# bcc-research/CFMMRouter.jl

Measured on AMD Instinct MI355X. Metric: find_arb! pools/sec + route! wall-clock, 1M-pool arbitrage, 1/2/4/8 GPU, higher is better.
Workload: dtype f64; 1 GPU; config3: 1M mixed ProductTwoCoin + GeometricMeanTwoCoin pools (500k each), 256 tokens, LinearNonnegative arbitrage; pools_per_gpu=1000000, pools_total=1000000, variant=materialising, full=False

## Files before the change

### cfmmrouter.jl_amd/csrc/sweep_core.h

```cpp
#pragma once

#include "granule.h"
#include "ops_two_coin.h"
#include "ops_univ3.h"

#include <type_traits>

namespace cfmm {

typedef double d2v __attribute__((ext_vector_type(2)));
__device__ __forceinline__ void store_pair(double2* dst, double x, double y, int nt)
{
    d2v val = {x, y};
    if (nt) asm volatile("global_store_dwordx4 %0, %1, off nt\n\ts_nop 1" : : "v"(dst), "v"(val) : "memory");
    else asm volatile("global_store_dwordx4 %0, %1, off sc1\n\ts_nop 1" : : "v"(dst), "v"(val) : "memory");
}
__device__ __forceinline__ void store_pair_at(double2* base, uint32_t i, double x, double y)
{
    d2v val = {x, y};
    asm volatile("s_nop 4\n\tglobal_store_dwordx4 %0, %1, %2 sc1\n\ts_nop 1" : : "v"(i * 16u), "v"(val), "s"(base) : "memory");
}

__device__ __forceinline__ void store_row(double* dst, double x)
{
    asm volatile("global_store_dwordx2 %0, %1, off sc1" : : "v"(dst), "v"(x) : "memory");
}

struct SweepLds {
    double2* vy;
    double2* gtab;
    double* lv;
    double* bins;
    double* wsum;
    double* flags;
    double* my_bins;
};

template <int BLOCK, bool GBINS>
__device__ __forceinline__ SweepLds carve_lds(const SweepArgs& a)
{
    extern __shared__ __attribute__((aligned(16))) double lds[];
    SweepLds L;
    if constexpr (GBINS) {
        L.vy = nullptr;
        L.gtab = nullptr;
        L.lv = L.bins = L.my_bins = L.flags = nullptr;
        L.wsum = lds;
        return L;
    }
    L.vy = reinterpret_cast<double2*>(lds);
    L.gtab = reinterpret_cast<double2*>(lds + ((size_t)a.n_pad << (a.v_shift - 3)));
    L.lv = reinterpret_cast<double*>(L.gtab + a.gtab_n);
    L.bins = L.lv + (a.need_logv ? a.n_pad : 0);
    L.wsum = L.bins + (size_t)a.copies * a.n_pad;
    L.flags = L.wsum + BLOCK / 64;
    L.my_bins = L.bins + (size_t)(a.copies == 1 ? 0 : (threadIdx.x >> 6)) * a.n_pad;
    return L;
}

__device__ __forceinline__ int wait_armed(const SweepArgs& a)
{
    const long long t0 = (long long)wall_clock64();
    for (;;) {
        const unsigned long long w = __hip_atomic_load(a.arm_word, __ATOMIC_RELAXED, __HIP_MEMORY_SCOPE_SYSTEM);
        if (w == a.arm_seq) return 1;
        if ((w & ~kArmCancel) > a.arm_seq || w == (a.arm_seq | kArmCancel)) return 0;
        if ((long long)wall_clock64() - t0 > a.arm_timeout) return -1;
        __builtin_amdgcn_s_sleep(1);
    }
}

__device__ __forceinline__ void report(const SweepArgs& a, unsigned long long bit)
{
    if (a.flags && threadIdx.x == 0) __hip_atomic_fetch_or(a.flags, bit, __ATOMIC_RELAXED, __HIP_MEMORY_SCOPE_SYSTEM);
}

constexpr int kStageLive = 1, kStageFast = 2, kStageGaveUp = 4;
constexpr int kPricePre = 2;
struct PricePre {
    double p[kPricePre];
};
template <int BLOCK>
__device__ __forceinline__ PricePre request_prices(const double* v, int n)
{
    PricePre r;
#pragma unroll
    for (int k = 0; k < kPricePre; ++k) {
        const int j = (int)threadIdx.x + k * BLOCK;
        r.p[k] = v[j < n ? j : n - 1];
    }
    return r;
}
template <int BLOCK, bool GBINS, bool PRE = false, bool LEAN = false>
__device__ __forceinline__ int stage_prices(const SweepArgs& a, const SweepLds& L, const PricePre& pre = PricePre{})
{
    if constexpr (GBINS) {
        __syncthreads();
        return kStageLive;
    }
    const int tid = threadIdx.x;
    const int n_zero = a.copies * a.n_pad;
    const bool logs = a.need_logv != 0;
    const bool armed = a.arm_word != nullptr;
    bool live = true, gave_up = false;
    if (armed) {
        for (int j = tid; j < n_zero; j += BLOCK) L.bins[j] = 0.0;
        for (int j = tid; j < a.gtab_n; j += BLOCK) {
            const double g = a.gtab[j];
            L.gtab[j] = make_double2(g, rcp_refined(g));
        }
        if (tid == 0) L.flags[BLOCK / 64] = (double)wait_armed(a);
        __syncthreads();
        live = L.flags[BLOCK / 64] > 0.0;
        gave_up = L.flags[BLOCK / 64] < 0.0;
    }
    bool in_window = true;
    for (int j = tid, k = 0; j < a.n; j += BLOCK, ++k) {
        double vj;
        if (armed) vj = __hip_atomic_load(a.v + j, __ATOMIC_RELAXED, __HIP_MEMORY_SCOPE_SYSTEM);
        else if (PRE && k < kPricePre) vj = k == 0 ? pre.p[0] : pre.p[1];
        else vj = a.v[j];
        if (a.v_shift == 4) L.vy[j] = make_double2(vj, rcp_refined(vj));
        else reinterpret_cast<double*>(L.vy)[j] = vj;
        in_window = in_window && in_fast_window(vj);
        if (logs) L.lv[j] = log(vj);
    }
    if (!armed) {
        for (int j = tid; j < n_zero; j += BLOCK) L.bins[j] = 0.0;
        for (int j = tid; j < a.gtab_n; j += BLOCK) {
            const double g = a.gtab[j];
            L.gtab[j] = make_double2(g, rcp_refined(g));
        }
    }
    const bool wave_in = __all(in_window ? 1 : 0) != 0;
    if ((tid & 63) == 0) L.flags[tid >> 6] = wave_in ? 1.0 : 0.0;
    __syncthreads();
    bool all_in = true;
    if constexpr (LEAN) {
        static_assert((BLOCK / 64) % 2 == 0, "flags are read in pairs");
        const double2* pairs = reinterpret_cast<const double2*>(L.flags);
        int bits = -1;
#pragma unroll
        for (int w = 0; w < BLOCK / 128; ++w) {
            const double2 f = pairs[w];
            bits &= __double2hiint(f.x) & __double2hiint(f.y);
        }
        all_in = bits != 0;
    } else {
#pragma unroll
        for (int w = 0; w < BLOCK / 64; ++w) all_in = all_in && L.flags[w] != 0.0;
    }
    return (live ? kStageLive : 0) | (all_in ? kStageFast : 0) | (gave_up ? kStageGaveUp : 0);
}

template <class Ops, bool MAT, bool GBINS, bool FAST, bool LEAN, class Idx>
__device__ __forceinline__ void finish_pool(const Ops& ops, const SweepArgs& a, const SweepLds& L, const typename Ops::Raw& raw,
                                            const Px& px, int2 tok, Idx i, double& acc)
{
    const auto put_record = [&](double x, double y) {
        if constexpr (LEAN) store_pair_at(a.Delta, i, x, y);
        else store_pair(a.Delta + i, x, y, a.nt_stores);
    };
    Trade t;
    double d, l;
    int dir;
    dir = ops.template solve_dir<FAST>(raw, px, d, l, t);
    const double v1 = px.v1, v2 = px.v2;
    const bool one = dir == kDir1 || dir == kDir2;
    const bool plain = one && (!MAT || !a.compact || (__double2hiint(d) | __double2hiint(l)) >= 0);
    if (plain) {
        const bool d1 = dir == kDir1;
        if (MAT) {
            if (a.compact) {
                put_record(d1 ? d : -d, l);
            } else {
                store_pair(a.Delta + i, d1 ? d : 0.0, d1 ? 0.0 : d, a.nt_stores);
                store_pair(a.Lambda + i, d1 ? 0.0 : l, d1 ? l : 0.0, a.nt_stores);
            }
        }
        acc += l * (d1 ? v2 : v1) - d * (d1 ? v1 : v2);
        if constexpr (GBINS) {
            a.gflow[i] = d1 ? make_double2(0.0 - d, l) : make_double2(l, 0.0 - d);
        } else {
            const double f_in = 0.0 - d;
            if (f_in != 0.0) atomicAdd(&L.my_bins[d1 ? tok.x : tok.y], f_in);
            if (l != 0.0) atomicAdd(&L.my_bins[d1 ? tok.y : tok.x], l);
        }
        return;
    }
    if (dir == kDirNone) {
        if (MAT) {
            if (a.compact) {
                put_record(0.0, 0.0);
            } else {
                store_pair(a.Delta + i, 0.0, 0.0, a.nt_stores);
                store_pair(a.Lambda + i, 0.0, 0.0, a.nt_stores);
            }
        }
        if constexpr (GBINS) a.gflow[i] = make_double2(0.0, 0.0);
        return;
    }
    expand_dir(dir, d, l, t);
    if (MAT) {
        if (a.compact) {
            const int d1h = __double2hiint(t.d1), d2h = __double2hiint(t.d2), l1h = __double2hiint(t.l1), l2h = __double2hiint(t.l2);
            const int z1 = d2h | __double2loint(t.d2) | l1h | __double2loint(t.l1);
            const int z2 = d1h | __double2loint(t.d1) | l2h | __double2loint(t.l2);
            const bool dir1 = (z1 == 0) & ((d1h | l2h) >= 0);
            const bool dir2 = (z2 == 0) & ((d2h | l1h) >= 0);
            double ra = t.d1, rb = t.l2;
            if (!dir1) {
                if (dir2) {
                    ra = -t.d2;
                    rb = t.l1;
                } else {
                    a.Lambda[i] = make_double2(t.d1, t.d2);
                    a.Over[i] = make_double2(t.l1, t.l2);
                    ra = 0.0;
                    rb = -1.0;
                }
            }
            put_record(ra, rb);
        } else {
            store_pair(a.Delta + i, t.d1, t.d2, a.nt_stores);
            store_pair(a.Lambda + i, t.l1, t.l2, a.nt_stores);
        }
    }
    acc += (t.l1 * v1 + t.l2 * v2) - (t.d1 * v1 + t.d2 * v2);
    const double f1 = t.l1 - t.d1, f2 = t.l2 - t.d2;
    if constexpr (GBINS) {
        a.gflow[i] = make_double2(f1, f2);
    } else {
        if (f1 != 0.0) atomicAdd(&L.my_bins[tok.x], f1);
        if (f2 != 0.0) atomicAdd(&L.my_bins[tok.y], f2);
    }
}

template <class Ops> struct HasLeanSolve : std::false_type {};
template <> struct HasLeanSolve<ProductOps> : std::true_type {};
template <> struct HasLeanSolve<GeoMeanLogOps> : std::true_type {};

template <class Ops, bool MAT, bool FAST, class Idx>
__device__ __forceinline__ void process_pool_lean(const Ops& ops, const SweepArgs& a, const SweepLds& L,
                                                  const typename Ops::Raw& raw_in, Idx i, double& acc)
{
    typename Ops::Raw raw = raw_in;
    const unsigned packed = (unsigned)raw.ai.x;
    const int2 tok = make_int2((int)(packed & 0xffffu), (int)(packed >> 16));
    const double2 gy = L.gtab[ops.p.gbase + raw.ai.y];
    const double2 a1 = L.vy[tok.x], a2 = L.vy[tok.y];
    double g = gy.x, yg = gy.y, v1 = a1.x, y1 = a1.y, v2 = a2.x, y2 = a2.y, lv1 = 0.0, lv2 = 0.0;
    if constexpr (Ops::kNeedsLogPrices) {
        lv1 = L.lv[tok.x];
        lv2 = L.lv[tok.y];
        asm volatile("" : "+v"(g), "+v"(yg), "+v"(v1), "+v"(y1), "+v"(v2), "+v"(y2), "+v"(lv1), "+v"(lv2));
    } else {
        asm volatile("" : "+v"(g), "+v"(yg), "+v"(v1), "+v"(y1), "+v"(v2), "+v"(y2));
    }
    raw.ai = tok;
    raw.g = g;
    raw.yg = yg;
    const Px px{v1, v2, y1, y2, yg, lv2 - lv1};
    double d, l;
    bool dir1, trades, rare;
    ops.template lean_solve<FAST>(raw, px, d, l, dir1, trades, rare);
    if (MAT) rare = rare | ((__double2hiint(d) | __double2hiint(l)) < 0);
    if (__builtin_expect(__any(rare ? 1 : 0) != 0, 0)) {
        finish_pool<Ops, MAT, false, FAST, true>(ops, a, L, raw, px, tok, i, acc);
        return;
    }
    if (MAT) store_pair_at(a.Delta, i, dir1 ? d : -d, l);
    const double worth = l * (dir1 ? v2 : v1) - d * (dir1 ? v1 : v2);
    acc = trades ? acc + worth : acc;
    const double f_in = 0.0 - d;
    if (f_in != 0.0) atomicAdd(&L.my_bins[dir1 ? tok.x : tok.y], f_in);
    if (l != 0.0) atomicAdd(&L.my_bins[dir1 ? tok.y : tok.x], l);
}

template <class Ops, bool MAT, bool GBINS, bool FAST, bool LEAN, class Idx>
__device__ __forceinline__ void process_pool(const Ops& ops, const SweepArgs& a, const SweepLds& L,
                                             const typename Ops::Raw& raw_in, Idx i, double& acc)
{
    if constexpr (LEAN && HasLeanSolve<Ops>::value) {
        process_pool_lean<Ops, MAT, FAST>(ops, a, L, raw_in, i, acc);
        return;
    }
    typename Ops::Raw raw = raw_in;
    ops.template resolve<GBINS, FAST, LEAN>(raw, L.gtab);
    const int2 tok = ops.tokens(raw);
    Px px;
    px.yg = raw.yg;
    if constexpr (GBINS) {
        px.v1 = a.v[tok.x];
        px.v2 = a.v[tok.y];
        px.y1 = px.y2 = 0.0;
        px.dlv = Ops::kNeedsLogPrices ? log(px.v2 / px.v1) : 0.0;
    } else {
        if constexpr (FAST) {
            const double2 a1 = L.vy[tok.x], a2 = L.vy[tok.y];
            px.v1 = a1.x; px.y1 = a1.y;
            px.v2 = a2.x; px.y2 = a2.y;
        } else {
            const char* base = reinterpret_cast<const char*>(L.vy);
            px.v1 = *reinterpret_cast<const double*>(base + ((size_t)tok.x << a.v_shift));
            px.v2 = *reinterpret_cast<const double*>(base + ((size_t)tok.y << a.v_shift));
            px.y1 = px.y2 = 0.0;
        }
        px.dlv = 0.0;
        if constexpr (Ops::kNeedsLogPrices)
            px.dlv = a.need_logv ? L.lv[tok.y] - L.lv[tok.x] : log(px.v2 / px.v1);
    }
    finish_pool<Ops, MAT, GBINS, FAST, LEAN>(ops, a, L, raw, px, tok, i, acc);
}

template <class Ops, bool MAT, int BLOCK, bool GBINS, bool FAST, bool PREFETCH, bool LEAN, class Idx>
__device__ __forceinline__ void tile_loop(const Ops& ops, const SweepArgs& a, const SweepLds& L, typename Ops::Raw cur,
                                          Idx i, Idx step, Idx left, double& acc)
{
    if constexpr (PREFETCH) {
        bool ok = left > 0;
        while (ok) {
            const bool more = left > 1;
            typename Ops::Raw nxt = cur;
            if (more) nxt = ops.template load<GBINS, LEAN>((Idx)(i + step));
            process_pool<Ops, MAT, GBINS, FAST, LEAN>(ops, a, L, cur, i, acc);
            i += step;
            --left;
            ok = more;
            cur = nxt;
        }
    } else {
        bool ok = left > 0;
        while (ok) {
            process_pool<Ops, MAT, GBINS, FAST, LEAN>(ops, a, L, cur, i, acc);
            i += step;
            ok = --left > 0;
            if (ok) cur = ops.template load<GBINS, LEAN>(i);
        }
    }
}

constexpr int kArithFull = 0, kArithFast = 1, kArithAuto = 2;
template <class Ops, bool MAT, int BLOCK, bool GBINS, int FASTK, bool MULTI, bool LEAN, class Idx>
__device__ __forceinline__ double sweep_tiles(const Ops& ops, const SweepArgs& a, const SweepLds& L, const typename Ops::Raw& cur,
                                              Idx i, Idx step, Idx left, bool& poison, bool& live, const PricePre& pre)
{
    static_assert(!(GBINS && FASTK != kArithFull), "large-market mode runs on the compiler's sequences");
    double acc = 0.0;
    const int staged = stage_prices<BLOCK, GBINS, !GBINS, LEAN>(a, L, pre);
    poison = (staged & kStageLive) == 0;
    live = !poison || (staged & kStageGaveUp) != 0;
    if (staged & kStageGaveUp) report(a, kFlagGaveUp);
    if (FASTK == kArithFast && !poison && (staged & kStageFast) == 0) {
        poison = true;
        report(a, kFlagWindow);
    }
    if (poison) left = 0;
    constexpr bool kPre = Ops::kPrefetch && !MULTI;
    if constexpr (FASTK == kArithAuto) {
        if (staged & kStageFast) tile_loop<Ops, MAT, BLOCK, GBINS, true, kPre, LEAN>(ops, a, L, cur, i, step, left, acc);
        else tile_loop<Ops, MAT, BLOCK, GBINS, false, kPre, LEAN>(ops, a, L, cur, i, step, left, acc);
    } else {
        tile_loop<Ops, MAT, BLOCK, GBINS, FASTK == kArithFast, kPre, LEAN>(ops, a, L, cur, i, step, left, acc);
    }
    return acc;
}

typedef unsigned long long u2v __attribute__((ext_vector_type(2)));
__device__ __forceinline__ void publish_column(const SweepArgs& a, int j, double val)
{
    if (a.direct_host.gran) {
        u2v g = {granule(a.direct_host.tag, val, 0), granule(a.direct_host.tag, val, 1)};
        asm volatile("global_store_dwordx4 %0, %1, off sc0 sc1\n\ts_nop 1" : : "v"(a.direct_host.gran + 2 * (size_t)j), "v"(g) : "memory");
    } else {
        a.direct_out[j] = val;
    }
}

template <int BLOCK, bool GBINS>
__device__ __forceinline__ void finish_row(const SweepArgs& a, const SweepLds& L, double acc, int row_id, bool poison, bool publish)
{
    const double nan = __builtin_nan("");
    if (poison) acc = nan;
    constexpr int kWaves = BLOCK / 64;
    const int tid = threadIdx.x;
    const int wave = tid >> 6;
#pragma unroll
    for (int off = 32; off > 0; off >>= 1) acc += __shfl_down(acc, off, 64);
    if ((tid & 63) == 0) L.wsum[wave] = acc;
    __syncthreads();

    const int n_cols = GBINS ? 0 : a.n;
    if (!GBINS && a.direct) {
        if (!publish) return;
        for (int j = tid; j < n_cols; j += BLOCK) {
            double s = L.bins[j];
            for (int c = 1; c < a.copies; ++c) s += L.bins[(size_t)c * a.n_pad + j];
            publish_column(a, j, poison ? nan : s);
        }
        if (tid == 0) {
            double s = L.wsum[0];
            for (int w = 1; w < kWaves; ++w) s += L.wsum[w];
            publish_column(a, n_cols, poison ? nan : s);
        }
        return;
    }
    double* row = a.partials + (size_t)row_id * a.row_pitch;
    for (int j = tid; j < n_cols; j += BLOCK) {
        double s = L.bins[j];
        for (int c = 1; c < a.copies; ++c) s += L.bins[(size_t)c * a.n_pad + j];
        store_row(row + j, poison ? nan : s);
    }
    if (tid == 0) {
        double s = L.wsum[0];
        for (int w = 1; w < kWaves; ++w) s += L.wsum[w];
        store_row(row + n_cols, poison ? nan : s);
    }
}

#define CFMM_CONST_AS __attribute__((address_space(4)))
template <class T>
__device__ __forceinline__ const CFMM_CONST_AS T* const_as(const T* p)
{
    return (const CFMM_CONST_AS T*)(reinterpret_cast<uintptr_t>(p));
}
struct LaunchHead {
    const SweepDesc* desc;
    const double* v;
    int reverse;
    int n;
};
static_assert(offsetof(SweepLaunch, desc) == 0 && offsetof(SweepLaunch, v) == 8 && offsetof(SweepLaunch, reverse) == 16 &&
                  offsetof(SweepLaunch, n) == 20 && offsetof(SweepLaunch, tail) == 24 && alignof(SweepTail) == 8,
              "sweep_kernel / sweep_multi (pointer, pointer, int, int, SweepTail) read the segment as a SweepLaunch");
typedef const CFMM_CONST_AS SweepLaunch& LaunchRef;
__device__ __forceinline__ LaunchRef launch_args()
{
    return *(const CFMM_CONST_AS SweepLaunch*)__builtin_amdgcn_kernarg_segment_ptr();
}
__device__ __forceinline__ BlockRec block_rec(const SweepDesc* desc)
{
    const CFMM_CONST_AS BlockRec* recs =
        (const CFMM_CONST_AS BlockRec*)(reinterpret_cast<uintptr_t>(desc) + kSweepDescHead);
    const CFMM_CONST_AS BlockRec& r = recs[blockIdx.x];
    return BlockRec{r.first, r.stride, r.full, r.tail, r.row, r.seg, r.kind};
}
__device__ __forceinline__ SweepArgs block_args(const LaunchHead& h, LaunchRef la, const CFMM_CONST_AS SweepDesc& d,
                                                const CFMM_CONST_AS SegRec& sg)
{
    const CFMM_CONST_AS SweepTail& t = la.tail;
    SweepArgs a;
    a.v = la.v;
    a.n = d.n;
    a.n_pad = d.n_pad;
    a.v_shift = d.v_shift;
    a.need_logv = d.need_logv;
    a.gtab = d.gtab;
    a.gtab_n = d.gtab_n;
    a.copies = d.copies;
    a.flags = d.flags;
    a.m = sg.m;
    a.Delta = sg.Delta;
    a.Lambda = sg.Lambda;
    a.Over = sg.Over;
    a.compact = d.compact;
    a.partials = d.partials;
    a.row_pitch = d.row_pitch;
    a.gflow = sg.gflow;
    a.reverse = h.reverse;
    a.arm_word = t.arm_word;
    a.arm_seq = t.arm_seq;
    a.arm_timeout = t.arm_timeout;
    a.nt_stores = d.nt_stores;
    a.direct = d.direct;
    a.direct_out = t.direct_out;
    a.direct_host = HostOut{t.direct_host.gran, t.direct_host.tag};
    return a;
}
__device__ __forceinline__ ProductPools pools_of(const CFMM_CONST_AS AnyPools& u, const ProductPools*)
{
    return ProductPools{u.p.R, u.p.gamma, u.p.Ai, u.p.pk, u.p.gbase};
}
__device__ __forceinline__ GeoMeanPools pools_of(const CFMM_CONST_AS AnyPools& u, const GeoMeanPools*)
{
    return GeoMeanPools{u.g.R, u.g.w, u.g.gamma, u.g.Ai, u.g.eta, u.g.Q, u.g.reference_order, u.g.pk, u.g.gbase};
}
__device__ __forceinline__ UniV3Pools pools_of(const CFMM_CONST_AS AnyPools& u, const UniV3Pools*)
{
    return UniV3Pools{u.u.pg, u.u.Ai, u.u.cur_a, u.u.cur_b, u.u.cur_c, u.u.curR, u.u.walk, u.u.ticks, u.u.thr, u.u.head,
                      u.u.has_walk, u.u.cp, u.u.pk, u.u.gbase};
}
template <class Ops, bool MAT, int BLOCK, bool GBINS, int FASTK, bool MULTI, bool LEAN>
__device__ __forceinline__ void sweep_body(const LaunchHead& h, const CFMM_CONST_AS SweepDesc& d, const CFMM_CONST_AS SegRec& sg,
                                           const BlockRec& br, const PricePre& pre)
{
    static_assert(!(LEAN && (GBINS || FASTK == kArithFull)), "the lean kernels: LDS bins, prices staged as pairs");
    using Idx = typename std::conditional<LEAN, uint32_t, int64_t>::type;
    const Ops ops{pools_of(sg.pools, (const decltype(Ops::p)*)nullptr)};
    const int64_t stride = br.stride;
    const int64_t i0 = br.first + threadIdx.x;
    const int64_t left = br.full + ((int)threadIdx.x < br.tail ? 1 : 0);
    const bool reverse = h.reverse != 0;
    const int64_t step = reverse ? -stride : stride;
    const int64_t i = reverse ? i0 + (left - 1) * stride : i0;
    typename Ops::Raw cur = {};
    if (left > 0) cur = ops.template load<GBINS, LEAN>((Idx)i);
    SweepArgs a = block_args(h, launch_args(), d, sg);
    if constexpr (LEAN) {
        a.compact = 1;
        a.nt_stores = 0;
        a.v_shift = 4;
        a.copies = BLOCK / 64;
        a.direct = 0;
    }
    const SweepLds L = carve_lds<BLOCK, GBINS>(a);
    if constexpr (LEAN) a.need_logv = Ops::kNeedsLogPrices ? 1 : 0;
    bool poison, live;
    const double acc = sweep_tiles<Ops, MAT, BLOCK, GBINS, FASTK, MULTI, LEAN>(ops, a, L, cur, (Idx)i, (Idx)step, (Idx)left, poison, live, pre);
    finish_row<BLOCK, GBINS>(a, L, acc, br.row, poison, live);
}

template <class Ops, bool MAT, int BLOCK, bool GBINS, int FASTK, bool LEAN = false>
__global__ __launch_bounds__(BLOCK) void sweep_kernel(const SweepDesc* desc, const double* v, int reverse, int n, SweepTail)
{
    const LaunchHead h{desc, v, reverse, n};
    PricePre pre = {};
    if constexpr (!GBINS) pre = request_prices<BLOCK>(v, n);
    const BlockRec br = block_rec(desc);
    const CFMM_CONST_AS SweepDesc& d = *const_as(desc);
    sweep_body<Ops, MAT, BLOCK, GBINS, FASTK, false, LEAN>(h, d, d.seg[0], br, pre);
}

template <bool MAT, int BLOCK, bool GBINS, int FASTK, bool LEAN = false>
__global__ __launch_bounds__(BLOCK) void sweep_multi(const SweepDesc* desc, const double* v, int reverse, int n, SweepTail)
{
    const LaunchHead h{desc, v, reverse, n};
    PricePre pre = {};
    if constexpr (!GBINS) pre = request_prices<BLOCK>(v, n);
    const BlockRec br = block_rec(desc);
    const CFMM_CONST_AS SweepDesc& d = *const_as(desc);
    const CFMM_CONST_AS SegRec& sg = d.seg[br.seg];
    switch (br.kind) {
    case 0: sweep_body<ProductOps, MAT, BLOCK, GBINS, FASTK, true, LEAN>(h, d, sg, br, pre); break;
    case 1:
        sweep_body<GeoMeanLogOps, MAT, BLOCK, GBINS, FASTK, true, LEAN>(h, d, sg, br, pre);
        break;
    default: sweep_body<UniV3Ops, MAT, BLOCK, GBINS, FASTK, true, LEAN>(h, d, sg, br, pre); break;
    }
}
#undef CFMM_CONST_AS

}
```

Measured before the change: 83.04 billion pools/s.

## Prefetch fee table at kernel entry and hand-schedule vmem waits in sweep loop

```diff
diff --git a/cfmmrouter.jl_amd/csrc/sweep_core.h b/cfmmrouter.jl_amd/csrc/sweep_core.h
--- a/cfmmrouter.jl_amd/csrc/sweep_core.h
+++ b/cfmmrouter.jl_amd/csrc/sweep_core.h
@@ -91,8 +91,22 @@
     }
     return r;
 }
+struct FeePre {
+    double g;
+};
+template <int BLOCK, bool LEAN>
+__device__ __forceinline__ FeePre request_fee(const double* gtab, int gtab_n)
+{
+    static_assert(kMaxFeeTable <= BLOCK, "the fee table is one entry per lane");
+    FeePre r = {1.0};
+    const int last = gtab_n - 1, j = (int)threadIdx.x;
+    if (LEAN || last >= 0) r.g = gtab[j < last ? j : last];
+    return r;
+}
+__device__ __forceinline__ void wait_vmem() { __builtin_amdgcn_s_waitcnt(0x0f70); }
 template <int BLOCK, bool GBINS, bool PRE = false, bool LEAN = false>
-__device__ __forceinline__ int stage_prices(const SweepArgs& a, const SweepLds& L, const PricePre& pre = PricePre{})
+__device__ __forceinline__ int stage_prices(const SweepArgs& a, const SweepLds& L, const PricePre& pre = PricePre{},
+                                            const FeePre& fee = FeePre{})
 {
     if constexpr (GBINS) {
         __syncthreads();
@@ -103,12 +117,19 @@
     const bool logs = a.need_logv != 0;
     const bool armed = a.arm_word != nullptr;
     bool live = true, gave_up = false;
+    const auto stage_fee = [&] {
+        if constexpr (PRE) {
+            if (tid < a.gtab_n) L.gtab[tid] = make_double2(fee.g, rcp_refined(fee.g));
+        } else {
+            for (int j = tid; j < a.gtab_n; j += BLOCK) {
+                const double g = a.gtab[j];
+                L.gtab[j] = make_double2(g, rcp_refined(g));
+            }
+        }
+    };
     if (armed) {
         for (int j = tid; j < n_zero; j += BLOCK) L.bins[j] = 0.0;
-        for (int j = tid; j < a.gtab_n; j += BLOCK) {
-            const double g = a.gtab[j];
-            L.gtab[j] = make_double2(g, rcp_refined(g));
-        }
+        stage_fee();
         if (tid == 0) L.flags[BLOCK / 64] = (double)wait_armed(a);
         __syncthreads();
         live = L.flags[BLOCK / 64] > 0.0;
@@ -117,8 +138,10 @@
     bool in_window = true;
     for (int j = tid, k = 0; j < a.n; j += BLOCK, ++k) {
         double vj;
-        if (armed) vj = __hip_atomic_load(a.v + j, __ATOMIC_RELAXED, __HIP_MEMORY_SCOPE_SYSTEM);
-        else if (PRE && k < kPricePre) vj = k == 0 ? pre.p[0] : pre.p[1];
+        if (armed) {
+            vj = __hip_atomic_load(a.v + j, __ATOMIC_RELAXED, __HIP_MEMORY_SCOPE_SYSTEM);
+            if constexpr (PRE) wait_vmem();
+        } else if (PRE && k < kPricePre) vj = k == 0 ? pre.p[0] : pre.p[1];
         else vj = a.v[j];
         if (a.v_shift == 4) L.vy[j] = make_double2(vj, rcp_refined(vj));
         else reinterpret_cast<double*>(L.vy)[j] = vj;
@@ -127,10 +150,7 @@
     }
     if (!armed) {
         for (int j = tid; j < n_zero; j += BLOCK) L.bins[j] = 0.0;
-        for (int j = tid; j < a.gtab_n; j += BLOCK) {
-            const double g = a.gtab[j];
-            L.gtab[j] = make_double2(g, rcp_refined(g));
-        }
+        stage_fee();
     }
     const bool wave_in = __all(in_window ? 1 : 0) != 0;
     if ((tid & 63) == 0) L.flags[tid >> 6] = wave_in ? 1.0 : 0.0;
@@ -317,25 +337,33 @@
 __device__ __forceinline__ void tile_loop(const Ops& ops, const SweepArgs& a, const SweepLds& L, typename Ops::Raw cur,
                                           Idx i, Idx step, Idx left, double& acc)
 {
+    wait_vmem();
     if constexpr (PREFETCH) {
         bool ok = left > 0;
-        while (ok) {
-            const bool more = left > 1;
+        for (;;) {
+            const bool more = ok && left > 1;
+            if (__any(more ? 1 : 0) == 0) break;
             typename Ops::Raw nxt = cur;
             if (more) nxt = ops.template load<GBINS, LEAN>((Idx)(i + step));
-            process_pool<Ops, MAT, GBINS, FAST, LEAN>(ops, a, L, cur, i, acc);
+            if (ok) process_pool<Ops, MAT, GBINS, FAST, LEAN>(ops, a, L, cur, i, acc);
             i += step;
             --left;
             ok = more;
             cur = nxt;
         }
+        if (MAT) __builtin_amdgcn_s_waitcnt(0x0f71);
+        else wait_vmem();
+        if (ok) process_pool<Ops, MAT, GBINS, FAST, LEAN>(ops, a, L, cur, i, acc);
     } else {
         bool ok = left > 0;
         while (ok) {
             process_pool<Ops, MAT, GBINS, FAST, LEAN>(ops, a, L, cur, i, acc);
             i += step;
             ok = --left > 0;
-            if (ok) cur = ops.template load<GBINS, LEAN>(i);
+            if (ok) {
+                cur = ops.template load<GBINS, LEAN>(i);
+                wait_vmem();
+            }
         }
     }
 }
@@ -343,11 +371,11 @@
 constexpr int kArithFull = 0, kArithFast = 1, kArithAuto = 2;
 template <class Ops, bool MAT, int BLOCK, bool GBINS, int FASTK, bool MULTI, bool LEAN, class Idx>
 __device__ __forceinline__ double sweep_tiles(const Ops& ops, const SweepArgs& a, const SweepLds& L, const typename Ops::Raw& cur,
-                                              Idx i, Idx step, Idx left, bool& poison, bool& live, const PricePre& pre)
+                                              Idx i, Idx step, Idx left, bool& poison, bool& live, const PricePre& pre, const FeePre& fee)
 {
     static_assert(!(GBINS && FASTK != kArithFull), "large-market mode runs on the compiler's sequences");
     double acc = 0.0;
-    const int staged = stage_prices<BLOCK, GBINS, !GBINS, LEAN>(a, L, pre);
+    const int staged = stage_prices<BLOCK, GBINS, !GBINS, LEAN>(a, L, pre, fee);
     poison = (staged & kStageLive) == 0;
     live = !poison || (staged & kStageGaveUp) != 0;
     if (staged & kStageGaveUp) report(a, kFlagGaveUp);
@@ -492,7 +520,7 @@
 }
 template <class Ops, bool MAT, int BLOCK, bool GBINS, int FASTK, bool MULTI, bool LEAN>
 __device__ __forceinline__ void sweep_body(const LaunchHead& h, const CFMM_CONST_AS SweepDesc& d, const CFMM_CONST_AS SegRec& sg,
-                                           const BlockRec& br, const PricePre& pre)
+                                           const BlockRec& br, const PricePre& pre, const FeePre& fee)
 {
     static_assert(!(LEAN && (GBINS || FASTK == kArithFull)), "the lean kernels: LDS bins, prices staged as pairs");
     using Idx = typename std::conditional<LEAN, uint32_t, int64_t>::type;
@@ -503,8 +531,8 @@
     const bool reverse = h.reverse != 0;
     const int64_t step = reverse ? -stride : stride;
     const int64_t i = reverse ? i0 + (left - 1) * stride : i0;
-    typename Ops::Raw cur = {};
-    if (left > 0) cur = ops.template load<GBINS, LEAN>((Idx)i);
+    const int64_t spare = (br.full | br.tail) != 0 ? br.first : 0;
+    const typename Ops::Raw cur = ops.template load<GBINS, LEAN>((Idx)(left > 0 ? i : spare));
     SweepArgs a = block_args(h, launch_args(), d, sg);
     if constexpr (LEAN) {
         a.compact = 1;
@@ -516,7 +544,7 @@
     const SweepLds L = carve_lds<BLOCK, GBINS>(a);
     if constexpr (LEAN) a.need_logv = Ops::kNeedsLogPrices ? 1 : 0;
     bool poison, live;
-    const double acc = sweep_tiles<Ops, MAT, BLOCK, GBINS, FASTK, MULTI, LEAN>(ops, a, L, cur, (Idx)i, (Idx)step, (Idx)left, poison, live, pre);
+    const double acc = sweep_tiles<Ops, MAT, BLOCK, GBINS, FASTK, MULTI, LEAN>(ops, a, L, cur, (Idx)i, (Idx)step, (Idx)left, poison, live, pre, fee);
     finish_row<BLOCK, GBINS>(a, L, acc, br.row, poison, live);
 }
 
@@ -528,7 +556,9 @@
     if constexpr (!GBINS) pre = request_prices<BLOCK>(v, n);
     const BlockRec br = block_rec(desc);
     const CFMM_CONST_AS SweepDesc& d = *const_as(desc);
-    sweep_body<Ops, MAT, BLOCK, GBINS, FASTK, false, LEAN>(h, d, d.seg[0], br, pre);
+    FeePre fee = {};
+    if constexpr (!GBINS) fee = request_fee<BLOCK, LEAN>(d.gtab, d.gtab_n);
+    sweep_body<Ops, MAT, BLOCK, GBINS, FASTK, false, LEAN>(h, d, d.seg[0], br, pre, fee);
 }
 
 template <bool MAT, int BLOCK, bool GBINS, int FASTK, bool LEAN = false>
@@ -539,13 +569,15 @@
     if constexpr (!GBINS) pre = request_prices<BLOCK>(v, n);
     const BlockRec br = block_rec(desc);
     const CFMM_CONST_AS SweepDesc& d = *const_as(desc);
+    FeePre fee = {};
+    if constexpr (!GBINS) fee = request_fee<BLOCK, LEAN>(d.gtab, d.gtab_n);
     const CFMM_CONST_AS SegRec& sg = d.seg[br.seg];
     switch (br.kind) {
-    case 0: sweep_body<ProductOps, MAT, BLOCK, GBINS, FASTK, true, LEAN>(h, d, sg, br, pre); break;
+    case 0: sweep_body<ProductOps, MAT, BLOCK, GBINS, FASTK, true, LEAN>(h, d, sg, br, pre, fee); break;
     case 1:
-        sweep_body<GeoMeanLogOps, MAT, BLOCK, GBINS, FASTK, true, LEAN>(h, d, sg, br, pre);
+        sweep_body<GeoMeanLogOps, MAT, BLOCK, GBINS, FASTK, true, LEAN>(h, d, sg, br, pre, fee);
         break;
-    default: sweep_body<UniV3Ops, MAT, BLOCK, GBINS, FASTK, true, LEAN>(h, d, sg, br, pre); break;
+    default: sweep_body<UniV3Ops, MAT, BLOCK, GBINS, FASTK, true, LEAN>(h, d, sg, br, pre, fee); break;
     }
 }
 #undef CFMM_CONST_AS
```

After: 83.29 billion pools/s (median of 5 runs). Within noise of the previous version (+0.3%).
